# morrislab/rnascan

Hardware: AMD Instinct MI355X
Metric: scored windows/sec (seq+struct, w=12) (higher is better)
Workload: dtype f64

## Files before the change

### include/pfmscan.h

```cpp
#ifndef PFMSCAN_H
#define PFMSCAN_H

#include <stdint.h>

#ifdef __cplusplus
extern "C" {
#endif

#define PFMSCAN_ABI_VERSION 18
#define PFMSCAN_NCODE   8
#define PFMSCAN_SEP     7
#define PFMSCAN_NSTRUCT 7
#define PFMSCAN_MAX_M   64
#define PFMSCAN_MAX_WIDTH 4096
#define PFMSCAN_SITE_GROUP 4096
#define PFMSCAN_SITE_LIMBS 66

#define PFMSCAN_OK          0
#define PFMSCAN_E_BADARG   -1
#define PFMSCAN_E_BADSHAPE -2
#define PFMSCAN_E_OOM      -3
#define PFMSCAN_E_HIP      -4
#define PFMSCAN_E_CAPACITY -5

#define PFMSCAN_PROFILE_NONE 0
#define PFMSCAN_PROFILE_F32  1
#define PFMSCAN_PROFILE_F64  2

typedef struct pfmscan_ctx pfmscan_ctx;
typedef struct pfmscan_motif pfmscan_motif;

int pfmscan_abi_version(void);
// ... 210 lines not shown
                                     int64_t *d_hit_pos, int32_t *d_hit_motif, float *d_hit_seq,
                                     double *d_hit_struct, uint64_t *d_hit_count, void *stream);
int pfmscan_library_hits_letters_host(pfmscan_ctx *ctx, pfmscan_library *lib,
                                      const uint8_t *codes, const uint8_t *codes2, int64_t n_pos,
                                      const double *thr_seq, const double *thr_struct, int64_t capacity,
                                      int64_t *hit_pos, int32_t *hit_motif, float *hit_seq,
                                      double *hit_struct, int64_t *n_hits);
int pfmscan_library_hits_letters_sum_dev(pfmscan_ctx *ctx, pfmscan_library *lib, const uint8_t *d_codes,
                                         const uint8_t *d_codes2, int64_t n_pos, const double *thr_seq,
                                         const double *thr_struct, const double *thr_sum, int64_t capacity,
                                         int64_t *d_hit_pos, int32_t *d_hit_motif, float *d_hit_seq,
                                         double *d_hit_struct, uint64_t *d_hit_count, void *stream);
int pfmscan_library_hits_letters_sum_host(pfmscan_ctx *ctx, pfmscan_library *lib, const uint8_t *codes,
                                          const uint8_t *codes2, int64_t n_pos, const double *thr_seq,
                                          const double *thr_struct, const double *thr_sum, int64_t capacity,
                                          int64_t *hit_pos, int32_t *hit_motif, float *hit_seq,
                                          double *hit_struct, int64_t *n_hits);
int pfmscan_library_letters_sum_thresholds(const double *letter_tables, const double *struct_tables, int n_motifs,
                                           int m, const double *thr_seq, const double *thr_sum, double *thr_eff);

int pfmscan_debug_credit_table(const double *letter_table, int m, double thr_seq, int bits,
                               uint16_t *credits, double *slack);

int pfmscan_debug_library8_credits(const double *letter_table, int m, double thr, uint16_t *credits, double *slack);

int pfmscan_debug_credit8_table(const double *letter_table, int m, double thr, uint16_t *credits, int *mode);

#define PFMSCAN_UPLOAD_RUNTIME 0
#define PFMSCAN_UPLOAD_STAGED  1
int pfmscan_set_upload_mode(pfmscan_ctx *ctx, int mode);
int pfmscan_upload_source_file(pfmscan_ctx *ctx, const void *base, size_t length, const char *path, int64_t file_offset);
int pfmscan_upload_source_file_checked(pfmscan_ctx *ctx, const void *base, size_t length, const char *path,
                                       int64_t file_offset, int64_t st_dev, int64_t st_ino, int64_t st_size);

int pfmscan_dotbracket_annotate_dev(pfmscan_ctx *ctx, const uint8_t *d_in, uint8_t *d_out, int64_t n_pos,
                                    const uint8_t *map, int64_t *d_counts, int64_t *first_bad, void *stream);
int pfmscan_dotbracket_stage(pfmscan_ctx *ctx, const uint8_t *codes, int64_t n_pos, int which, const uint8_t *map,
                             int64_t *counts, int64_t *first_bad);
int pfmscan_dotbracket_annotate_host(pfmscan_ctx *ctx, const uint8_t *in, uint8_t *out, int64_t n_pos,
                                     const uint8_t *map, int64_t *counts, int64_t *first_bad);

#define PFMSCAN_MAX_COVER 1024
#define PFMSCAN_AVG_OK         0
#define PFMSCAN_AVG_DOTBRACKET 1
#define PFMSCAN_AVG_UNCOVERED  2
#define PFMSCAN_AVG_COVER      3
// ... 117 lines not shown
```

### rnascan_amd/_lib.py

```python
import ctypes
import importlib.util
import os
import sys

import numpy as np

HERE = os.path.dirname(os.path.abspath(__file__))
LIB_PATH = os.environ.get("PFMSCAN_LIB") or os.path.join(HERE, "libpfmscan.so")

OK = 0
E_BADARG, E_BADSHAPE, E_OOM, E_HIP, E_CAPACITY = -1, -2, -3, -4, -5
PROFILE_NONE, PROFILE_F32, PROFILE_F64 = 0, 1, 2
SEP = 7
NCODE = 8
NSTRUCT = 7
MAX_M = 64
MAX_WIDTH = 4096
ABI_VERSION = 18

SYMBOLS = [
    "pfmscan_abi_version", "pfmscan_ctx_create", "pfmscan_ctx_destroy", "pfmscan_last_error",
    "pfmscan_device_info", "pfmscan_synchronize", "pfmscan_motif_create", "pfmscan_motif_destroy",
    "pfmscan_pwm_calculate", "pfmscan_scan_dev", "pfmscan_scan_letters_f64_dev", "pfmscan_hits_dev",
    "pfmscan_scan_host", "pfmscan_scan_letters_f64_host", "pfmscan_hits_host", "pfmscan_time_scan_dev",
    "pfmscan_stage", "pfmscan_scan_staged", "pfmscan_hits_staged", "pfmscan_hits_adaptive_dev",
    "pfmscan_library_create", "pfmscan_library_destroy", "pfmscan_library_info", "pfmscan_library_hits_dev",
    "pfmscan_library_hits_staged", "pfmscan_library_hits_host", "pfmscan_library_hits_pipeline_host", "pfmscan_debug_credit_table",
    "pfmscan_library_create_letters", "pfmscan_library_hits_letters_dev", "pfmscan_library_hits_letters_host", "pfmscan_debug_library8_credits",
    "pfmscan_debug_credit8_table",
    "pfmscan_hits_pipeline_host", "pfmscan_staged_positions",
    "pfmscan_hits_letters_f64_dev", "pfmscan_hits_letters_f64_staged", "pfmscan_hits_letters_f64_host",
    "pfmscan_hits_pair_dev", "pfmscan_stage_codes2", "pfmscan_hits_pair_staged", "pfmscan_hits_pair_host", "pfmscan_round_decimals",
    "pfmscan_set_upload_mode", "pfmscan_upload_source_file", "pfmscan_upload_source_file_checked", "pfmscan_fasta_lone_cr", "pfmscan_count_bytes", "pfmscan_fasta_index", "pfmscan_fasta_ids", "pfmscan_gather_spans", "pfmscan_fasta_encode", "pfmscan_tsv_format", "pfmscan_profile_parse", "pfmscan_tsv_number",
    "pfmscan_place_alloc", "pfmscan_place_free", "pfmscan_place_note", "pfmscan_place_trim",
    "pfmscan_dotbracket_annotate_dev", "pfmscan_dotbracket_stage", "pfmscan_dotbracket_annotate_host",
    "pfmscan_average_dev", "pfmscan_average_host", "pfmscan_average_stage", "pfmscan_fragment_ids",
    "pfmscan_profile_colsums_dev", "pfmscan_profile_colsums_host", "pfmscan_profile_colsums_staged",
    "pfmscan_hits_sum_dev", "pfmscan_hits_sum_staged", "pfmscan_hits_sum_host", "pfmscan_hits_sum_pipeline_host",
    "pfmscan_library_hits_sum_dev", "pfmscan_library_hits_sum_staged", "pfmscan_library_hits_sum_host",
    "pfmscan_profile_row_bound_dev", "pfmscan_profile_row_bound_staged", "pfmscan_library_sum_thresholds",
    "pfmscan_site_groups", "pfmscan_site_sums_dev", "pfmscan_site_sums_staged", "pfmscan_site_sums_host",
    "pfmscan_site_groups_lib", "pfmscan_site_order_lib", "pfmscan_site_acc_add", "pfmscan_site_acc_round",
    "pfmscan_site_acc_from_doubles", "pfmscan_site_sums_lib_dev", "pfmscan_site_sums_lib_staged",
    "pfmscan_hits_pair_sum_dev", "pfmscan_hits_pair_sum_staged", "pfmscan_hits_pair_sum_host", "pfmscan_pair_sum_route",
    "pfmscan_debug_round3d", "pfmscan_debug_pair_sum_test", "pfmscan_debug_pair_credits",
    "pfmscan_library_hits_letters_sum_dev", "pfmscan_library_hits_letters_sum_host", "pfmscan_library_letters_sum_thresholds",
    "pfmscan_library_last_launches",
]
PAIR_ROUTE_NONE, PAIR_ROUTE_FUSED, PAIR_ROUTE_TWO_PHASE, PAIR_ROUTE_DENSE, PAIR_ROUTE_CREDITS = range(5)
SITE_GROUP = 4096
SITE_LIMBS = 66
MAX_COVER = 1024
AVG_OK, AVG_DOTBRACKET, AVG_UNCOVERED, AVG_COVER, AVG_BAD_TABLE = range(5)
TSV_CONST, TSV_I64, TSV_F32, TSV_F64, TSV_INDEXED, TSV_FIXED, TSV_WINDOW, TSV_SPAN = range(8)


class TsvColumn(ctypes.Structure):
    _fields_ = [("kind", ctypes.c_int32), ("reserved", ctypes.c_int32), ("data", ctypes.c_void_p),
                ("aux", ctypes.c_void_p), ("blob", ctypes.c_void_p), ("width", ctypes.c_int64)]



class CapacityError(RuntimeError):

    def __init__(self, msg, required):
        RuntimeError.__init__(self, msg)
        self.required = required


_lib = None
# ... 111 lines not shown
    L.pfmscan_place_trim.argtypes = [vp]
    L.pfmscan_place_note.argtypes = [vp]
    L.pfmscan_place_note.restype = ctypes.c_char_p
    L.pfmscan_fasta_index.argtypes = [vp, i64, i64, vp, vp, vp, vp, vp, ctypes.POINTER(i64), i32]
    L.pfmscan_fasta_ids.argtypes = [vp, vp, vp, i64, vp, vp, ctypes.POINTER(i32)]
    L.pfmscan_gather_spans.argtypes = [vp, vp, i64, i32, vp, i64, ctypes.POINTER(i64)]
    L.pfmscan_fasta_encode.argtypes = [vp, vp, vp, vp, i64, i64, vp, i32, vp, vp, i32]
    L.pfmscan_profile_parse.argtypes = [ctypes.c_char_p, i64, i32, i64, vp, ctypes.POINTER(i64)]
    L.pfmscan_tsv_number.argtypes = [vp, i64, i64, vp, i64, ctypes.POINTER(i64), ctypes.POINTER(i64), ctypes.POINTER(i32)]
    L.pfmscan_hits_letters_f64_dev.argtypes = [vp, vp, vp, i64, dbl, i64, vp, vp, vp, vp]
    L.pfmscan_hits_letters_f64_staged.argtypes = [vp, vp, dbl, i64, vp, vp, ctypes.POINTER(i64)]
    L.pfmscan_hits_letters_f64_host.argtypes = [vp, vp, vp, i64, dbl, i64, vp, vp, ctypes.POINTER(i64)]
    L.pfmscan_hits_pair_dev.argtypes = [vp, vp, vp, vp, vp, i64, dbl, dbl, i64, vp, vp, vp, vp, vp]
    L.pfmscan_stage_codes2.argtypes = [vp, vp, i64]
    L.pfmscan_hits_pair_staged.argtypes = [vp, vp, vp, dbl, dbl, i64, vp, vp, vp, ctypes.POINTER(i64)]
    L.pfmscan_hits_pair_host.argtypes = [vp, vp, vp, vp, vp, i64, dbl, dbl, i64, vp, vp, vp, ctypes.POINTER(i64)]
    L.pfmscan_round_decimals.argtypes = [vp, i64, i32, vp, i32]
    L.pfmscan_hits_pair_sum_dev.argtypes = [vp, vp, vp, vp, vp, i64, dbl, dbl, dbl, i64, vp, vp, vp, vp, vp]
    L.pfmscan_hits_pair_sum_staged.argtypes = [vp, vp, vp, dbl, dbl, dbl, i64, vp, vp, vp, ctypes.POINTER(i64)]
    L.pfmscan_hits_pair_sum_host.argtypes = [vp, vp, vp, vp, vp, i64, dbl, dbl, dbl, i64, vp, vp, vp, ctypes.POINTER(i64)]
    L.pfmscan_pair_sum_route.argtypes = [vp]
    L.pfmscan_library_last_launches.argtypes = [vp, ctypes.POINTER(i32), ctypes.POINTER(i32), ctypes.POINTER(i32)]
    L.pfmscan_debug_round3d.argtypes = [vp, i64, vp]
    L.pfmscan_library_hits_letters_sum_dev.argtypes = [vp, vp, vp, vp, i64, vp, vp, vp, i64, vp, vp, vp, vp, vp, vp]
    L.pfmscan_library_hits_letters_sum_host.argtypes = [vp, vp, vp, vp, i64, vp, vp, vp, i64, vp, vp, vp, vp, ctypes.POINTER(i64)]
    L.pfmscan_library_letters_sum_thresholds.argtypes = [vp, vp, i32, i32, vp, vp, vp]
    L.pfmscan_debug_pair_credits.argtypes = [vp, vp, i32, dbl, vp, vp] + [ctypes.POINTER(dbl)] * 4 + [ctypes.POINTER(i32)]
    L.pfmscan_debug_pair_sum_test.argtypes = [vp, vp, i64, dbl, vp, vp, ctypes.POINTER(dbl)]
    L.pfmscan_tsv_format.argtypes = [ctypes.POINTER(TsvColumn), i32, i64, i64, vp, i64, ctypes.POINTER(i64), vp, ctypes.POINTER(i32), i32]
    for name in SYMBOLS:
        if name not in ("pfmscan_ctx_destroy", "pfmscan_motif_destroy", "pfmscan_last_error", "pfmscan_library_destroy",
                        "pfmscan_staged_positions", "pfmscan_place_note"):
            getattr(L, name).restype = i32
    L.pfmscan_staged_positions.restype = i64
    if L.pfmscan_abi_version() != ABI_VERSION:
        raise ImportError("libpfmscan ABI %d, bindings expect %d" % (L.pfmscan_abi_version(), ABI_VERSION))
    _lib = L
    return L


def _ptr(a):
    if a is None:
        return None
    if isinstance(a, np.ndarray):
        return a.ctypes.data_as(ctypes.c_void_p)
    return ctypes.c_void_p(int(a))
# ... 1296 lines not shown
    tj = np.ascontiguousarray(np.broadcast_to(np.asarray(thr_sum, dtype=np.float64), (n,)))
    out = np.empty(n, dtype=np.float64)
    rc = L.pfmscan_library_sum_thresholds(_ptr(T), _ptr(P), n, m, _ptr(ts), _ptr(tj), float(row_sum_max), _ptr(out))
    if rc != OK:
        raise ValueError("pfmscan_library_sum_thresholds: bad argument")
    return out


def library8_credits(letter_table, thr):
    L = load()
    T = np.ascontiguousarray(letter_table, dtype=np.float64)
    if T.ndim != 2 or T.shape[1] != NCODE:
        raise ValueError("letter_table must be [m][8]")
    rows = (T.shape[0] + 3) // 4 * 4
    out = np.zeros((rows, 8), dtype=np.uint16)
    slack = ctypes.c_double(0.0)
    L.pfmscan_debug_library8_credits.argtypes = [ctypes.c_void_p, ctypes.c_int, ctypes.c_double, ctypes.c_void_p, ctypes.POINTER(ctypes.c_double)]
    rc = L.pfmscan_debug_library8_credits(_ptr(T), T.shape[0], float(thr), _ptr(out), ctypes.byref(slack))
    if rc != OK:
        raise ValueError("pfmscan_debug_library8_credits: bad argument")
    return out, slack.value


def credit8_table(letter_table, thr):
    L = load()
    T = np.ascontiguousarray(letter_table, dtype=np.float64)
    if T.ndim != 2 or T.shape[1] != NCODE:
        raise ValueError("letter_table must be [m][8]")
    out = np.zeros((T.shape[0], 8), dtype=np.uint16)
    mode = ctypes.c_int(0)
    rc = L.pfmscan_debug_credit8_table(_ptr(T), T.shape[0], float(thr), _ptr(out), ctypes.byref(mode))
    if rc != OK:
        raise ValueError("pfmscan_debug_credit8_table: bad argument")
    return out, mode.value


def _stream_args(motif, codes, profile):
    if motif.has_letters:
        if codes is None:
            raise ValueError("motif has a letter table: codes required")
        codes = np.ascontiguousarray(codes, dtype=np.uint8)
        n = codes.size
    dt = PROFILE_NONE
    if motif.has_struct:
        if profile is None:
            raise ValueError("motif has a structure PSSM: profile required")
# ... 16 lines not shown
```

### rnascan_amd/csrc/pfmscan_exact.hpp

```cpp
#pragma once
#include <float.h>
#include <math.h>
#include <algorithm>
#include <cmath>
#include <hip/hip_runtime.h>

namespace pfmscan {

constexpr double STRUCT_ROW_MAX = 1024.0;

inline double struct_band(const double *pssm, int m)
{
    double s = 0.0;
    for (int i = 0; i < m * 7; ++i)
        if (std::isfinite(pssm[i])) s += std::fabs(pssm[i]);
    return 24.0 * (double)m * 0x1p-53 * STRUCT_ROW_MAX * s;
}

__device__ __forceinline__ double exact_nan_to_num(double d)
{
    const double c = fmin(fmax(d, -DBL_MAX), DBL_MAX);
    return (d != d) ? 0.0 : c;
}

template <typename ROW_T, typename CellF>
__device__ __forceinline__ double struct_window_rounded(const ROW_T *rows, int m, CellF cell)
{
#pragma clang fp contract(off)
    double score = 0.0;
#pragma unroll 1
    for (int j = 0; j < m; ++j) {
        double d = 0.0;
#pragma unroll 1
        for (int k = 0; k < 7; ++k) {
            const double prod = (double)rows[j * 7 + k] * cell(j, k);
            d = d + prod;
        }
        score = score + exact_nan_to_num(d);
    }
// ... 174 lines not shown
```

### rnascan_amd/csrc/pfmscan_internal.hpp

```cpp
#pragma once
#include <hip/hip_runtime.h>
#include <stdint.h>
#include <atomic>
#include "../../include/pfmscan.h"

namespace pfmscan {

struct CredCache {
    double thr = __builtin_nan("");
    int mode = 0;
    uint16_t cr[16 * 16];
};

struct Cred8Cache {
    double thr = __builtin_nan("");
    int mode = 0;
    uint16_t cr[32 * 8];
};

struct PairCred {
    int mode = 0;
    int m = 0;
    double thr_sum = __builtin_nan("");
    double thr_joint = 0.0, quantum = 0.0, slack = 0.0, survive = 0.0;
// ... 146 lines not shown
    const double *thr_sum;
};
size_t lib_group_bytes(int m, int npair, bool has_struct, int np_bucket);
size_t lib_queue_bytes(int np_bucket);
size_t lib_lds_bytes(int m, int npair, int ng, bool has_struct, int np_bucket);
int lib_np_bucket(int m);
int lib_pick_ng(int np_bucket, int want_groups, int max_groups);
hipError_t launch_library(const LibArgs &a, int n_cu, hipStream_t stream);
constexpr int PROFILE_LETTERS2 = 100;
__host__ __device__ constexpr int lib8_rows(int m) { return (m + 3) / 4 * 4; }
size_t lib8_group_bytes(int m);
size_t lib8_lds_bytes(int m, int ng);
int lib8_pick_ng(int want_groups, int max_groups);
hipError_t launch_library8(const LibArgs &a, int n_cu, hipStream_t stream);

struct ProfLibArgs {
    const void *profile;
    int profile_dtype;
    int64_t n_pos;
    const double *pssm;
    const double *thr;
    double struct_band;
    const int32_t *finite;
    int n_motifs, m, motif_base;
    int64_t pos_offset;
    int64_t capacity;
    int hit_shards;
    int64_t *hit_pos;
    int32_t *hit_motif;
    double *hit_struct;
    unsigned long long *hit_count;
};
hipError_t launch_profile_library(const ProfLibArgs &a, hipStream_t stream);
int64_t profile_library_tile();

hipError_t sort_temp_bytes(int64_t total, int key_bits, size_t *bytes);
hipError_t launch_gather_sorted(const GatherArgs &g, hipStream_t stream);

}
```

### rnascan_amd/csrc/pfmscan_library_api.hip

```cpp
#include <algorithm>
#include <cmath>
#include <cstdlib>
#include <cstring>
#include <new>
#include <string>
#include <vector>

#include "pfmscan_hits.hpp"

using namespace pfmscan;

namespace {

struct LibPass {
    int motif_base = 0, n_real = 0, nmp = 0, ng = 0;
    int ng_real = 0;
    size_t pairs_off = 0;
    size_t letters_off = 0;
    size_t pssm_off = 0;
    size_t thr_off = 0;
};

}

// ... 46 lines not shown
        }
    return q * npair;
}

void pfmscan::pair_sums(const double *T, int m, double *out)
{
    const int npair = (m + 1) / 2;
    for (int t = 0; t < npair; ++t)
        for (int c0 = 0; c0 < 4; ++c0)
            for (int c1 = 0; c1 < 4; ++c1)
                out[t * 16 + (c0 | c1 << 2)] = T[(2 * t) * 8 + c0] + (2 * t + 1 < m ? T[(2 * t + 1) * 8 + c1] : 0.0);
}

struct pfmscan_library {
    pfmscan_ctx *ctx = nullptr;
    int n = 0, m = 0, npair = 0, np_bucket = 8;
    bool has_struct = false;
    bool has_letters = true;
    bool pair = false;
    bool letters8 = false;
    std::vector<double> rows8;
    double *d_pssm_rows = nullptr;
    int32_t *d_finite = nullptr;
    bool all_finite = false;
    double struct_band = 0.0;
    std::vector<double> pairsum;
    std::vector<LibPass> passes;
    uint16_t *d_pairs = nullptr;
    double *d_letters = nullptr, *d_pssm = nullptr, *d_thr = nullptr;
    size_t pairs_elems = 0, thr_elems = 0;
    std::vector<uint16_t> h_pairs;
    std::vector<double> h_thr;
    std::vector<double> cur_seq, cur_struct, eps;
    std::vector<double> h_letters, h_pssm;
    std::vector<double> band;
    std::vector<double> cur_eff, cur_sum;
    bool thr_valid = false;
    int last_launches = 0, last_team_launches = 0, last_max_teams = 0;
};

static int lib_fail(pfmscan_ctx *ctx, int code, const std::string &msg) { return fail(ctx, code, msg); }

extern "C" {

static int create_seq_library(pfmscan_ctx *ctx, const double *letter_tables, const double *struct_pssms, int ncol, int n_motifs, int m,
                              pfmscan_library **out);
// ... 1 lines not shown
int pfmscan_library_create(pfmscan_ctx *ctx, const double *letter_tables, const double *struct_pssms, int n_motifs, int m,
                           pfmscan_library **out)
{
    if (!ctx || !out || (!letter_tables && !struct_pssms)) return lib_fail(ctx, PFMSCAN_E_BADARG, "pfmscan_library_create: NULL argument");
    *out = nullptr;
    if (n_motifs < 1 || n_motifs > 65535) return lib_fail(ctx, PFMSCAN_E_BADSHAPE, "library size outside 1..65535");
    if (m < 1 || m > PFMSCAN_MAX_M)
        return lib_fail(ctx, PFMSCAN_E_BADSHAPE, "PFM width " + std::to_string(m) + " outside 1.." + std::to_string(PFMSCAN_MAX_M));
    if (!letter_tables) {
        HIP_TRY(ctx, hipSetDevice(ctx->device));
        pfmscan_library *lib = new (std::nothrow) pfmscan_library();
        if (!lib) return lib_fail(ctx, PFMSCAN_E_OOM, "out of host memory");
        lib->ctx = ctx;
        lib->n = n_motifs;
        lib->m = m;
        lib->has_struct = true;
        lib->has_letters = false;
        for (int k = 0; k < n_motifs; ++k) lib->struct_band = std::max(lib->struct_band, struct_band(struct_pssms + (size_t)k * m * 7, m));
        std::vector<int32_t> fin((size_t)n_motifs, 1);
        for (int k = 0; k < n_motifs; ++k)
            for (int i = 0; i < m * 7; ++i)
                if (!std::isfinite(struct_pssms[(size_t)k * m * 7 + i])) fin[(size_t)k] = 0;
        if (std::getenv("PFMSCAN_FORCE_GENERIC")) std::fill(fin.begin(), fin.end(), 0);
        const size_t cells = (size_t)n_motifs * m * 7;
        hipError_t e = hipMalloc((void **)&lib->d_pssm_rows, cells * 8);
        if (e == hipSuccess) e = hipMemcpy(lib->d_pssm_rows, struct_pssms, cells * 8, hipMemcpyHostToDevice);
        if (e == hipSuccess) e = hipMalloc((void **)&lib->d_finite, (size_t)n_motifs * 4);
        if (e == hipSuccess) e = hipMemcpy(lib->d_finite, fin.data(), (size_t)n_motifs * 4, hipMemcpyHostToDevice);
        if (e == hipSuccess) e = hipMalloc((void **)&lib->d_thr, (size_t)n_motifs * 8);
        lib->thr_elems = (size_t)n_motifs;
        if (e != hipSuccess) {
            pfmscan_library_destroy(lib);
            return fail_hip(ctx, e, "uploading the library tables");
        }
        *out = lib;
        return PFMSCAN_OK;
    }
    return create_seq_library(ctx, letter_tables, struct_pssms, 7, n_motifs, m, out);
}

}

static int create_seq_library(pfmscan_ctx *ctx, const double *letter_tables, const double *struct_pssms, int ncol, int n_motifs, int m,
                              pfmscan_library **out)
{
    for (int64_t i = 0; i < (int64_t)n_motifs * m; ++i)
        for (int c = 4; c < 8; ++c)
            if (!std::isnan(letter_tables[i * 8 + c]))
// ... 160 lines not shown
{
    if (!ctx || !out || !struct_tables) return lib_fail(ctx, PFMSCAN_E_BADARG, "pfmscan_library_create_letters: NULL argument");
    *out = nullptr;
    if (n_motifs < 1 || n_motifs > 65535) return lib_fail(ctx, PFMSCAN_E_BADSHAPE, "library size outside 1..65535");
    if (m < 1 || m > PFMSCAN_MAX_M)
        return lib_fail(ctx, PFMSCAN_E_BADSHAPE, "PFM width " + std::to_string(m) + " outside 1.." + std::to_string(PFMSCAN_MAX_M));
    for (int64_t i = 0; i < (int64_t)n_motifs * m; ++i)
        if (!std::isnan(struct_tables[i * 8 + 7]))
            return lib_fail(ctx, PFMSCAN_E_BADSHAPE, "column 7 of every letter table must be NaN (the foreign code)");
    if (seq_tables) return create_seq_library(ctx, seq_tables, struct_tables, 8, n_motifs, m, out);
    return create_letters8_library(ctx, struct_tables, n_motifs, m, out);
}

void pfmscan_library_destroy(pfmscan_library *lib)
{
    if (!lib) return;
    if (lib->ctx) (void)hipSetDevice(lib->ctx->device);
    if (lib->d_pairs) (void)hipFree(lib->d_pairs);
    if (lib->d_letters) (void)hipFree(lib->d_letters);
    if (lib->d_pssm) (void)hipFree(lib->d_pssm);
    if (lib->d_thr) (void)hipFree(lib->d_thr);
    if (lib->d_pssm_rows) (void)hipFree(lib->d_pssm_rows);
    if (lib->d_finite) (void)hipFree(lib->d_finite);
    delete lib;
}

int pfmscan_debug_credit_table(const double *letter_table, int m, double thr_seq, int bits, uint16_t *credits, double *slack)
{
    if (!letter_table || !credits || m < 1 || m > PFMSCAN_MAX_M || std::isnan(thr_seq)) return PFMSCAN_E_BADARG;
    if (bits == 0) bits = lib_credit_bits(lib_np_bucket(m));
    if (bits != 10 && bits != 16) return PFMSCAN_E_BADARG;
    const int npair = (m + 1) / 2;
    std::vector<double> ps((size_t)npair * 16);
    pair_sums(letter_table, m, ps.data());
    const double s = build_credits(ps.data(), npair, thr_seq, credits, bits);
    if (slack) *slack = s;
    return PFMSCAN_OK;
}

int pfmscan_debug_library8_credits(const double *letter_table, int m, double thr, uint16_t *credits, double *slack)
{
    if (!letter_table || !credits || m < 1 || m > 32 || std::isnan(thr)) return PFMSCAN_E_BADARG;
    const int rows = lib8_rows(m);
    std::vector<double> r8((size_t)rows * 8, 0.0);
    for (int j = 0; j < m; ++j)
        for (int c = 0; c < 8; ++c) r8[(size_t)j * 8 + c] = std::isnan(letter_table[j * 8 + c]) ? -INFINITY : letter_table[j * 8 + c];
    const double s = build_credits(r8.data(), rows, thr, credits, 16, 8);
    if (slack) *slack = s;
    return PFMSCAN_OK;
}

int pfmscan_library_info(const pfmscan_library *lib, int *n_motifs, int *m, int *n_passes, int *motifs_per_pass, double *max_eps)
{
    if (!lib) return PFMSCAN_E_BADARG;
    if (n_motifs) *n_motifs = lib->n;
    if (m) *m = lib->m;
    const bool tabled = lib->has_letters || lib->letters8;
    if (n_passes) *n_passes = tabled ? (int)lib->passes.size() : 1;
    if (motifs_per_pass) *motifs_per_pass = !tabled ? lib->n : (lib->passes.empty() ? 0 : lib->passes[0].nmp);
    if (max_eps) {
        double mx = 0.0;
        for (double v : lib->eps) mx = std::max(mx, v);
        *max_eps = lib->thr_valid ? mx : NAN;
    }
    return PFMSCAN_OK;
}

int pfmscan_library_last_launches(const pfmscan_library *lib, int *n_launches, int *n_team_launches, int *max_teams)
{
    if (!lib) return PFMSCAN_E_BADARG;
    if (n_launches) *n_launches = lib->last_launches;
// ... 161 lines not shown
                a.capacity = sink.shard_cap;
                a.hit_shards = sink.shards;
                a.hit_pos = sink.pos;
                a.hit_motif = sink.motif;
                a.hit_seq = nullptr;
                a.hit_struct = sink.st;
                a.hit_count = sink.count;
                hipError_t e = launch_library8(a, ctx->n_cu, st);
                if (e != hipSuccess) return fail_hip(ctx, e, "launch k_library8");
                lib_note_launch(lib, 1);
            }
        return PFMSCAN_OK;
    }
    if (!lib->has_letters) {
        ProfLibArgs a;
        std::memset(&a, 0, sizeof(a));
        a.profile = d_profile;
        a.profile_dtype = profile_dtype;
        a.n_pos = n_pos;
        a.pssm = lib->d_pssm_rows;
        a.thr = lib->d_thr;
        a.struct_band = lib->struct_band;
        a.finite = lib->d_finite;
        a.n_motifs = lib->n;
        a.m = lib->m;
        a.motif_base = 0;
        a.pos_offset = pos_offset;
        a.capacity = sink.shard_cap;
        a.hit_shards = sink.shards;
        a.hit_pos = sink.pos;
        a.hit_motif = sink.motif;
        a.hit_struct = sink.st;
        a.hit_count = sink.count;
        hipError_t e = launch_profile_library(a, st);
        if (e != hipSuccess) return fail_hip(ctx, e, "launch k_profile_lib");
        lib_note_launch(lib, 1);
        return PFMSCAN_OK;
    }
    const LibPass &first_pass = lib->passes[0];
    bool teams = lib->has_struct && !lib->pair && lib->passes.size() > 1 && n_pos >= (int64_t)8 * ctx->n_cu * LIB_SEG &&
                 ctx->n_cu >= 16 && !std::getenv("PFMSCAN_LIB_SEQUENTIAL");
    for (const LibPass &ps : lib->passes) teams = teams && ps.ng == first_pass.ng;
    const int64_t max_span = (int64_t)1 << 31;
    for (int64_t base = 0; base < n_pos; base += max_span) {
        const int64_t span_segs = (std::min<int64_t>(max_span, n_pos - base) + LIB_SEG - 1) / LIB_SEG;
        const size_t per_launch = teams && span_segs >= ctx->n_cu ? 4 : 1;
// ... 424 lines not shown
```

### rnascan_amd/csrc/pfmscan_proflib.hip

```cpp
#include <float.h>
#include <math.h>

#include "pfmscan_internal.hpp"
#include "pfmscan_exact.hpp"
#include "pfmscan_hitqueue.hpp"

namespace pfmscan {

constexpr int PL_LANES = 256;
constexpr int PL_GROUPS = 4;
constexpr int PL_BLOCK = PL_LANES * PL_GROUPS;
#ifndef PL_V_OVERRIDE
#define PL_V_OVERRIDE 5
#endif
constexpr int PL_V = PL_V_OVERRIDE;
constexpr int PL_NS = PL_V + 1;
constexpr int PL_UNROLL = (PL_NS % 2) ? 2 * PL_NS : PL_NS;
constexpr int PL_TILE = PL_LANES * PL_V;
#ifndef PL_WAIT_FIRST
#define PL_WAIT_FIRST 1
#endif
#ifndef PL_STAGGER
#define PL_STAGGER 0
#endif
#ifndef PL_INTERLEAVE
#define PL_INTERLEAVE 0
#endif
constexpr int PL_QCAP = 128;

typedef uint32_t pl_u32x4 __attribute__((ext_vector_type(4)));
typedef double pl_f64x2 __attribute__((ext_vector_type(2)));

__device__ __forceinline__ double pl_nan_to_num(double d)
{
    double c = fmin(fmax(d, -DBL_MAX), DBL_MAX);
    return (d != d) ? 0.0 : c;
}

__host__ __device__ constexpr int pl_tile_vals(int m) { return ((PL_TILE + m) * 7 + 3) / 4 * 4; }
__host__ __device__ constexpr int pl_tile_bytes(int m) { return pl_tile_vals(m) * 8; }
__host__ __device__ constexpr int pl_queue_bytes() { return (PL_BLOCK / 64) * PL_QCAP * (8 + 4); }

__device__ __forceinline__ double pl_window_slow(const double *tile, int local, const double *__restrict__ pssm, int m)
{
    double score = 0.0;
#pragma unroll 1
    for (int j = 0; j < m; ++j) {
        const double *r = tile + (local + j) * 7;
        double d = r[0] * pssm[j * 7];
#pragma unroll 1
        for (int k = 1; k < 7; ++k) d = fma(r[k], pssm[j * 7 + k], d);
        score += pl_nan_to_num(d);
    }
    return score;
}

template <bool FINITE>
__device__ __forceinline__ void pl_score_motif(const double *tile, const double *__restrict__ pssm, const double *__restrict__ pssm_next,
                                               int m, int la, double (&acc)[PL_V], double (&P)[7])
{
    constexpr int V = PL_V, NS = PL_NS;
    const volatile __attribute__((address_space(3))) double *vt = (const volatile __attribute__((address_space(3))) double *)tile;
    double rows[NS][7];
#pragma unroll
// ... 47 lines not shown
            }
        }
    };
    int j0 = 0;
#pragma unroll 1
    for (; j0 + PL_UNROLL <= m; j0 += PL_UNROLL) {
#pragma unroll
        for (int uu = 0; uu < PL_UNROLL; ++uu) step(uu, j0 + uu);
    }
#pragma unroll
    for (int uu = 0; uu < PL_UNROLL - 1; ++uu) {
        if (j0 + uu < m) step(uu, j0 + uu);
    }
    if (m & 1) {
#pragma unroll
        for (int k = 0; k < 7; ++k) P[k] = Q[k];
    }
    if (FINITE) {
#pragma unroll
        for (int v = 0; v < V; ++v)
            if (!(fabs(acc[v]) <= DBL_MAX)) acc[v] = pl_window_slow(tile, la + v, pssm, m);
    }
}

template <typename PROF_T>
__global__ __launch_bounds__(PL_BLOCK) void k_profile_lib(const ProfLibArgs a)
{
    constexpr int V = PL_V;
    constexpr int PER = 16 / (int)sizeof(PROF_T);
    typedef PROF_T vec_t __attribute__((ext_vector_type(PER)));
    extern __shared__ __align__(16) unsigned char smem[];
    const int m = a.m;
    double *tile = reinterpret_cast<double *>(smem);
    const int lane = threadIdx.x & 63;
    const int wave = __builtin_amdgcn_readfirstlane(threadIdx.x >> 6);
    const int group = wave / (PL_LANES / 64);
    double *q_sc = reinterpret_cast<double *>(smem + pl_tile_bytes(m)) + wave * PL_QCAP;
    uint32_t *q_wm = reinterpret_cast<uint32_t *>(smem + pl_tile_bytes(m) + (PL_BLOCK / 64) * PL_QCAP * 8) + wave * PL_QCAP;
    const int64_t n_pos = a.n_pos;
    const int64_t tile0 = (int64_t)blockIdx.x * PL_TILE;

    {
        const int nval = pl_tile_vals(m);
        const int64_t e0 = tile0 * 7, e_end = n_pos * 7;
        const PROF_T *__restrict__ src = reinterpret_cast<const PROF_T *>(a.profile) + e0;
        for (int i = threadIdx.x * PER; i < nval; i += PL_BLOCK * PER) {
            double d[PER];
            if (e0 + i + PER <= e_end) {
                const vec_t v = __builtin_nontemporal_load(reinterpret_cast<const vec_t *>(src + i));
#pragma unroll
                for (int e = 0; e < PER; ++e) d[e] = (double)v[e];
            } else {
#pragma unroll
                for (int e = 0; e < PER; ++e) d[e] = (e0 + i + e < e_end) ? (double)src[i + e] : 0.0;
            }
#pragma unroll
            for (int e = 0; e < PER; e += 2) *reinterpret_cast<pl_f64x2 *>(tile + i + e) = pl_f64x2{d[e], d[e + 1]};
        }
    }
    if (threadIdx.x < PL_LANES / 64)
        reinterpret_cast<uint32_t *>(smem + pl_tile_bytes(m) + pl_queue_bytes())[threadIdx.x] = PL_GROUPS;
    __syncthreads();
#if PL_STAGGER
    if (group == 1) __builtin_amdgcn_s_sleep(PL_STAGGER);
    if (group == 2) __builtin_amdgcn_s_sleep(2 * PL_STAGGER);
    if (group == 3) __builtin_amdgcn_s_sleep(3 * PL_STAGGER);
#endif

    const HitShard shard{a.hit_count, a.hit_shards, a.capacity};
    const unsigned long long shard_off = shard.off();
    int qn = 0;
    auto flush = [&]() {
        __builtin_amdgcn_fence(__ATOMIC_RELEASE, "wavefront");
        __builtin_amdgcn_wave_barrier();
        __builtin_amdgcn_fence(__ATOMIC_ACQUIRE, "wavefront");
        const unsigned long long base = shard.reserve_wave(qn);
        for (int i = lane; i < qn; i += 64) {
            const unsigned long long slot = base + (unsigned long long)i;
            if (shard.in_range(slot)) {
                const uint32_t wm = q_wm[i];
                a.hit_pos[shard_off + slot] = tile0 + (int64_t)(wm >> 16) + a.pos_offset;
                a.hit_motif[shard_off + slot] = a.motif_base + (int32_t)(wm & 0xFFFFu);
                a.hit_struct[shard_off + slot] = q_sc[i];
            }
        }
        __builtin_amdgcn_fence(__ATOMIC_RELEASE, "wavefront");
        __builtin_amdgcn_wave_barrier();
        qn = 0;
    };

    const int la = (threadIdx.x & (PL_LANES - 1)) * V;
    const int64_t live_all = n_pos - m + 1 - tile0;
    const int live_n = live_all < 0 ? 0 : (live_all > PL_TILE ? PL_TILE : (int)live_all);
    const __attribute__((address_space(4))) double *thr = (const __attribute__((address_space(4))) double *)a.thr;
    const __attribute__((address_space(4))) int32_t *finite = (const __attribute__((address_space(4))) int32_t *)a.finite;

    uint32_t *ticket = reinterpret_cast<uint32_t *>(smem + pl_tile_bytes(m) + pl_queue_bytes()) + (wave & (PL_LANES / 64 - 1));
    auto draw = [&]() -> uint32_t {
        uint32_t v = 0;
        if (lane == 0) v = atomicAdd(ticket, 1u);
        return v;
    };
    const int nm = a.n_motifs;
    int k = group;
    int kn = nm;
    double P[7];
    int fin = 0;
    if (k < nm) {
        const __attribute__((address_space(4))) double *p0 = (const __attribute__((address_space(4))) double *)(a.pssm + (size_t)k * m * 7);
#pragma unroll
        for (int c = 0; c < 7; ++c) P[c] = p0[c];
        fin = finite[k];
        kn = (int)__builtin_amdgcn_readfirstlane(draw());
    }
#pragma unroll 1
    while (k < nm) {
        const double *pssm = a.pssm + (size_t)k * m * 7;
        const int kc = kn < nm ? kn : k;
        const double *pssm_next = a.pssm + (size_t)kc * m * 7;
        const double t = thr[k];
        const int fin_next = finite[kc];
        double acc[V];
        if (fin)
            pl_score_motif<true>(tile, pssm, pssm_next, m, la, acc, P);
        else
            pl_score_motif<false>(tile, pssm, pssm_next, m, la, acc, P);
        fin = fin_next;
        const double t_lo = t - a.struct_band, t_hi = t + a.struct_band;
        bool maybe[V], any = false;
#pragma unroll
        for (int v = 0; v < V; ++v) {
            maybe[v] = (la + v < live_n) && (acc[v] > t_lo);
            any = any || maybe[v];
        }
        if (__builtin_expect(__builtin_amdgcn_ballot_w64(any) != 0, 0)) {
#pragma unroll
            for (int v = 0; v < V; ++v) {
                bool pass = maybe[v];
                if (__builtin_amdgcn_ballot_w64(pass) == 0) continue;
                if (pass && acc[v] <= t_hi) {
                    acc[v] = struct_window_rounded(tile + (la + v) * 7, m, [&](int j, int c) { return pssm[j * 7 + c]; });
                    pass = acc[v] > t;
                }
                const unsigned long long mk = __builtin_amdgcn_ballot_w64(pass);
                if (mk) {
                    if (qn + 64 > PL_QCAP) flush();
                    if (pass) {
                        const int slot = qn + (int)__builtin_amdgcn_mbcnt_hi((uint32_t)(mk >> 32), __builtin_amdgcn_mbcnt_lo((uint32_t)mk, 0u));
                        q_sc[slot] = acc[v];
                        q_wm[slot] = ((uint32_t)(la + v) << 16) | (uint32_t)k;
                    }
                    qn += __popcll(mk);
                }
            }
        }
        k = kn;
        if (kn < nm) kn = (int)__builtin_amdgcn_readfirstlane(draw());
    }
    if (qn > 0) flush();
}

int64_t profile_library_tile() { return PL_TILE; }

hipError_t launch_profile_library(const ProfLibArgs &a, hipStream_t stream)
{
    if (a.n_pos <= 0 || a.n_motifs <= 0) return hipSuccess;
    if (a.n_motifs > 65536 || a.m < 1 || a.m > PFMSCAN_MAX_M) return hipErrorInvalidValue;
    const unsigned grid = (unsigned)((a.n_pos + PL_TILE - 1) / PL_TILE);
    const size_t lds = (size_t)pl_tile_bytes(a.m) + pl_queue_bytes() + 16;
    static std::atomic<uint64_t> done_f{0}, done_d{0};
    if (a.profile_dtype == PFMSCAN_PROFILE_F64) {
        hipError_t e = allow_dynamic_lds(reinterpret_cast<const void *>(k_profile_lib<double>), done_d, 160 * 1024);
        if (e != hipSuccess) return e;
        hipLaunchKernelGGL(k_profile_lib<double>, dim3(grid), dim3(PL_BLOCK), lds, stream, a);
    } else {
        hipError_t e = allow_dynamic_lds(reinterpret_cast<const void *>(k_profile_lib<float>), done_f, 160 * 1024);
        if (e != hipSuccess) return e;
        hipLaunchKernelGGL(k_profile_lib<float>, dim3(grid), dim3(PL_BLOCK), lds, stream, a);
    }
    return hipGetLastError();
}

}
```

Measured before the change: 151.8 billion.

## Add f32 screening pass with rigorous error bound to skip f64 struct scoring

Adds a float32 screening pass over the profile-library kernel. Each tile also gets an f32 copy of the structure profile in LDS, and each motif gets a host-computed error-bound coefficient, so a motif whose screened scores cannot exceed the threshold is skipped without the f64 scoring loop. An adaptive rule turns the screen off for a wave when most screens end up needing the f64 rerun. The cost is extra LDS use (which may lower occupancy), extra tile-conversion work, and a duplicate pass for motifs that survive the screen.

```diff
diff --git a/include/pfmscan.h b/include/pfmscan.h
--- a/include/pfmscan.h
+++ b/include/pfmscan.h
@@ -7,7 +7,7 @@
 extern "C" {
 #endif
 
-#define PFMSCAN_ABI_VERSION 18
+#define PFMSCAN_ABI_VERSION 19
 #define PFMSCAN_NCODE   8
 #define PFMSCAN_SEP     7
 #define PFMSCAN_NSTRUCT 7
@@ -264,6 +264,9 @@
 int pfmscan_debug_credit_table(const double *letter_table, int m, double thr_seq, int bits,
                                uint16_t *credits, double *slack);
 
+int pfmscan_debug_proflib_screen(const void *rows, int64_t n_rows, int row_is_f64, const double *pssm, int m,
+                                 float *s32_out, double *acc64_out, double *A_out);
+
 int pfmscan_debug_library8_credits(const double *letter_table, int m, double thr, uint16_t *credits, double *slack);
 
 int pfmscan_debug_credit8_table(const double *letter_table, int m, double thr, uint16_t *credits, int *mode);
diff --git a/rnascan_amd/_lib.py b/rnascan_amd/_lib.py
--- a/rnascan_amd/_lib.py
+++ b/rnascan_amd/_lib.py
@@ -16,7 +16,7 @@
 NSTRUCT = 7
 MAX_M = 64
 MAX_WIDTH = 4096
-ABI_VERSION = 18
+ABI_VERSION = 19
 
 SYMBOLS = [
     "pfmscan_abi_version", "pfmscan_ctx_create", "pfmscan_ctx_destroy", "pfmscan_last_error",
@@ -45,7 +45,7 @@
     "pfmscan_hits_pair_sum_dev", "pfmscan_hits_pair_sum_staged", "pfmscan_hits_pair_sum_host", "pfmscan_pair_sum_route",
     "pfmscan_debug_round3d", "pfmscan_debug_pair_sum_test", "pfmscan_debug_pair_credits",
     "pfmscan_library_hits_letters_sum_dev", "pfmscan_library_hits_letters_sum_host", "pfmscan_library_letters_sum_thresholds",
-    "pfmscan_library_last_launches",
+    "pfmscan_library_last_launches", "pfmscan_debug_proflib_screen",
 ]
 PAIR_ROUTE_NONE, PAIR_ROUTE_FUSED, PAIR_ROUTE_TWO_PHASE, PAIR_ROUTE_DENSE, PAIR_ROUTE_CREDITS = range(5)
 SITE_GROUP = 4096
@@ -203,6 +203,7 @@
     L.pfmscan_pair_sum_route.argtypes = [vp]
     L.pfmscan_library_last_launches.argtypes = [vp, ctypes.POINTER(i32), ctypes.POINTER(i32), ctypes.POINTER(i32)]
     L.pfmscan_debug_round3d.argtypes = [vp, i64, vp]
+    L.pfmscan_debug_proflib_screen.argtypes = [vp, i64, i32, vp, i32, vp, vp, ctypes.POINTER(dbl)]
     L.pfmscan_library_hits_letters_sum_dev.argtypes = [vp, vp, vp, vp, i64, vp, vp, vp, i64, vp, vp, vp, vp, vp, vp]
     L.pfmscan_library_hits_letters_sum_host.argtypes = [vp, vp, vp, vp, i64, vp, vp, vp, i64, vp, vp, vp, vp, ctypes.POINTER(i64)]
     L.pfmscan_library_letters_sum_thresholds.argtypes = [vp, vp, i32, i32, vp, vp, vp]
@@ -1545,6 +1546,24 @@
     return out, slack.value
 
 
+def debug_proflib_screen(rows, pssm):
+    L = load()
+    P = np.ascontiguousarray(pssm, dtype=np.float64)
+    if P.ndim != 2 or P.shape[1] != NSTRUCT:
+        raise ValueError("pssm must be [m][7]")
+    R = np.ascontiguousarray(rows)
+    if R.dtype not in (np.float32, np.float64) or R.ndim != 2 or R.shape[1] != NSTRUCT:
+        raise ValueError("rows must be float32 or float64 [n][7]")
+    n_win = max(0, R.shape[0] - P.shape[0] + 1)
+    s32, acc = np.zeros(n_win, dtype=np.float32), np.zeros(n_win, dtype=np.float64)
+    A = ctypes.c_double(0.0)
+    rc = L.pfmscan_debug_proflib_screen(_ptr(R), R.shape[0], int(R.dtype == np.float64), _ptr(P), P.shape[0], _ptr(s32), _ptr(acc),
+                                        ctypes.byref(A))
+    if rc != OK:
+        raise ValueError("pfmscan_debug_proflib_screen: bad argument")
+    return s32, acc, A.value
+
+
 def credit8_table(letter_table, thr):
     L = load()
     T = np.ascontiguousarray(letter_table, dtype=np.float64)
diff --git a/rnascan_amd/csrc/pfmscan_exact.hpp b/rnascan_amd/csrc/pfmscan_exact.hpp
--- a/rnascan_amd/csrc/pfmscan_exact.hpp
+++ b/rnascan_amd/csrc/pfmscan_exact.hpp
@@ -15,6 +15,54 @@
     for (int i = 0; i < m * 7; ++i)
         if (std::isfinite(pssm[i])) s += std::fabs(pssm[i]);
     return 24.0 * (double)m * 0x1p-53 * STRUCT_ROW_MAX * s;
+}
+
+typedef float scr_f32x2 __attribute__((ext_vector_type(2)));
+
+__host__ __device__ constexpr int screen_roundings(int m) { return 8 * m + 1; }
+__host__ __device__ __forceinline__ double screen_floor(int m) { return (double)screen_roundings(m) * 0x1p-149; }
+
+inline double screen_A(const double *pssm, int m)
+{
+    double s = 0.0;
+    for (int i = 0; i < m * 7; ++i) {
+        const double a = std::fabs(pssm[i]);
+        if (!(a <= (double)FLT_MAX) || (a != 0.0 && a < 0x1p-126)) return INFINITY;
+        s = std::nextafter(s + a, INFINITY);
+    }
+    const double n3 = (double)(screen_roundings(m) + 3);
+    const double c32 = std::nextafter(std::nextafter(n3 * 0x1p-24, INFINITY) * (1.0 + 0x1p-20), INFINITY);
+    const double coef = std::nextafter(c32 + (double)(7 * m + 1) * 0x1p-53, INFINITY);
+    const double A = std::nextafter(coef * s, INFINITY);
+    return std::isfinite(A) ? A : INFINITY;
+}
+
+template <typename T>
+__host__ __device__ __forceinline__ float screen_mag_up(T v)
+{
+    const double a = fabs((double)v);
+    if (!(a <= DBL_MAX)) return INFINITY;
+    float f = (float)a;
+    if ((double)f < a) f = __builtin_bit_cast(float, __builtin_bit_cast(uint32_t, f) + 1u);
+    return f;
+}
+
+__host__ __device__ __forceinline__ void screen_row_fma(scr_f32x2 &acc, const scr_f32x2 (&row)[4], const scr_f32x2 (&c)[4])
+{
+#pragma unroll
+    for (int q = 0; q < 4; ++q) acc = __builtin_elementwise_fma(row[q], c[q], acc);
+}
+__host__ __device__ __forceinline__ float screen_finish(scr_f32x2 acc)
+{
+#pragma clang fp contract(off)
+    return acc.x + acc.y;
+}
+__host__ __device__ __forceinline__ double screen_E(float M, double A, int m) { return fma((double)fmaxf(M, FLT_MIN), A, screen_floor(m)); }
+__host__ __device__ __forceinline__ bool screen_survives(float s32, double E, double t_lo)
+{
+#pragma clang fp contract(off)
+    const double d = (double)s32 + E;
+    return !(d <= t_lo && s32 >= -FLT_MAX);
 }
 
 __device__ __forceinline__ double exact_nan_to_num(double d)
diff --git a/rnascan_amd/csrc/pfmscan_internal.hpp b/rnascan_amd/csrc/pfmscan_internal.hpp
--- a/rnascan_amd/csrc/pfmscan_internal.hpp
+++ b/rnascan_amd/csrc/pfmscan_internal.hpp
@@ -192,6 +192,8 @@
     const double *thr;
     double struct_band;
     const int32_t *finite;
+    const float *pssm32;
+    const double *screen_a;
     int n_motifs, m, motif_base;
     int64_t pos_offset;
     int64_t capacity;
diff --git a/rnascan_amd/csrc/pfmscan_library_api.hip b/rnascan_amd/csrc/pfmscan_library_api.hip
--- a/rnascan_amd/csrc/pfmscan_library_api.hip
+++ b/rnascan_amd/csrc/pfmscan_library_api.hip
@@ -92,6 +92,8 @@
     std::vector<double> rows8;
     double *d_pssm_rows = nullptr;
     int32_t *d_finite = nullptr;
+    float *d_pssm32 = nullptr;
+    double *d_screen_a = nullptr;
     bool all_finite = false;
     double struct_band = 0.0;
     std::vector<double> pairsum;
@@ -139,8 +141,23 @@
             for (int i = 0; i < m * 7; ++i)
                 if (!std::isfinite(struct_pssms[(size_t)k * m * 7 + i])) fin[(size_t)k] = 0;
         if (std::getenv("PFMSCAN_FORCE_GENERIC")) std::fill(fin.begin(), fin.end(), 0);
+        std::vector<float> p32((size_t)n_motifs * m * 8, 0.0f);
+        std::vector<double> scr_a((size_t)n_motifs, INFINITY);
+        for (int k = 0; k < n_motifs; ++k) {
+            const double *P = struct_pssms + (size_t)k * m * 7;
+            if (fin[(size_t)k]) scr_a[(size_t)k] = screen_A(P, m);
+            if (scr_a[(size_t)k] < INFINITY) {
+                fin[(size_t)k] |= 2;
+                for (int j = 0; j < m; ++j)
+                    for (int c = 0; c < 7; ++c) p32[((size_t)k * m + j) * 8 + c] = (float)P[j * 7 + c];
+            }
+        }
         const size_t cells = (size_t)n_motifs * m * 7;
         hipError_t e = hipMalloc((void **)&lib->d_pssm_rows, cells * 8);
+        if (e == hipSuccess) e = hipMalloc((void **)&lib->d_pssm32, p32.size() * 4);
+        if (e == hipSuccess) e = hipMemcpy(lib->d_pssm32, p32.data(), p32.size() * 4, hipMemcpyHostToDevice);
+        if (e == hipSuccess) e = hipMalloc((void **)&lib->d_screen_a, (size_t)n_motifs * 8);
+        if (e == hipSuccess) e = hipMemcpy(lib->d_screen_a, scr_a.data(), (size_t)n_motifs * 8, hipMemcpyHostToDevice);
         if (e == hipSuccess) e = hipMemcpy(lib->d_pssm_rows, struct_pssms, cells * 8, hipMemcpyHostToDevice);
         if (e == hipSuccess) e = hipMalloc((void **)&lib->d_finite, (size_t)n_motifs * 4);
         if (e == hipSuccess) e = hipMemcpy(lib->d_finite, fin.data(), (size_t)n_motifs * 4, hipMemcpyHostToDevice);
@@ -347,6 +364,8 @@
     if (lib->d_thr) (void)hipFree(lib->d_thr);
     if (lib->d_pssm_rows) (void)hipFree(lib->d_pssm_rows);
     if (lib->d_finite) (void)hipFree(lib->d_finite);
+    if (lib->d_pssm32) (void)hipFree(lib->d_pssm32);
+    if (lib->d_screen_a) (void)hipFree(lib->d_screen_a);
     delete lib;
 }
 
@@ -372,6 +391,44 @@
         for (int c = 0; c < 8; ++c) r8[(size_t)j * 8 + c] = std::isnan(letter_table[j * 8 + c]) ? -INFINITY : letter_table[j * 8 + c];
     const double s = build_credits(r8.data(), rows, thr, credits, 16, 8);
     if (slack) *slack = s;
+    return PFMSCAN_OK;
+}
+
+int pfmscan_debug_proflib_screen(const void *rows, int64_t n_rows, int row_is_f64, const double *pssm, int m,
+                                 float *s32_out, double *acc64_out, double *A_out)
+{
+    if (!rows || !pssm || !s32_out || !acc64_out || !A_out || m < 1 || m > PFMSCAN_MAX_M || n_rows < 0) return PFMSCAN_E_BADARG;
+    *A_out = screen_A(pssm, m);
+    std::vector<scr_f32x2> c((size_t)m * 4);
+    for (int j = 0; j < m; ++j)
+        for (int q = 0; q < 4; ++q) {
+            const double lo = pssm[j * 7 + 2 * q], hi = 2 * q + 1 < 7 ? pssm[j * 7 + 2 * q + 1] : 0.0;
+            auto cvt = [](double v) { return std::isfinite(v) && std::fabs(v) > (double)FLT_MAX ? (float)std::copysign(INFINITY, v) : (float)v; };
+            c[(size_t)j * 4 + q] = scr_f32x2{cvt(lo), cvt(hi)};
+        }
+    auto entry = [&](int64_t r, int col) -> double {
+        return row_is_f64 ? static_cast<const double *>(rows)[r * 7 + col] : (double)static_cast<const float *>(rows)[r * 7 + col];
+    };
+    auto entry32 = [&](int64_t r, int col) -> float {
+        if (col >= 7) return 0.0f;
+        const double v = entry(r, col);
+        return std::isfinite(v) && std::fabs(v) > (double)FLT_MAX ? (float)std::copysign(INFINITY, v) : (float)v;
+    };
+    for (int64_t i = 0; i + m <= n_rows; ++i) {
+        scr_f32x2 acc = {0.0f, 0.0f};
+        double acc64 = 0.0;
+        for (int j = 0; j < m; ++j) {
+            scr_f32x2 row[4], cj[4];
+            for (int q = 0; q < 4; ++q) {
+                row[q] = scr_f32x2{entry32(i + j, 2 * q), entry32(i + j, 2 * q + 1)};
+                cj[q] = c[(size_t)j * 4 + q];
+            }
+            screen_row_fma(acc, row, cj);
+            for (int col = 0; col < 7; ++col) acc64 = std::fma(entry(i + j, col), pssm[j * 7 + col], acc64);
+        }
+        s32_out[i] = screen_finish(acc);
+        acc64_out[i] = acc64;
+    }
     return PFMSCAN_OK;
 }
 
@@ -579,6 +636,11 @@
         a.thr = lib->d_thr;
         a.struct_band = lib->struct_band;
         a.finite = lib->d_finite;
+        {
+            static const bool screen_on = !(std::getenv("PFMSCAN_PROFLIB_SCREEN") && std::getenv("PFMSCAN_PROFLIB_SCREEN")[0] == '0');
+            a.pssm32 = screen_on ? lib->d_pssm32 : nullptr;
+            a.screen_a = screen_on ? lib->d_screen_a : nullptr;
+        }
         a.n_motifs = lib->n;
         a.m = lib->m;
         a.motif_base = 0;
diff --git a/rnascan_amd/csrc/pfmscan_proflib.hip b/rnascan_amd/csrc/pfmscan_proflib.hip
--- a/rnascan_amd/csrc/pfmscan_proflib.hip
+++ b/rnascan_amd/csrc/pfmscan_proflib.hip
@@ -40,6 +40,11 @@
 __host__ __device__ constexpr int pl_tile_vals(int m) { return ((PL_TILE + m) * 7 + 3) / 4 * 4; }
 __host__ __device__ constexpr int pl_tile_bytes(int m) { return pl_tile_vals(m) * 8; }
 __host__ __device__ constexpr int pl_queue_bytes() { return (PL_BLOCK / 64) * PL_QCAP * (8 + 4); }
+__host__ __device__ constexpr int pl_tickets_bytes() { return 16; }
+__host__ __device__ constexpr int pl_wavemax_bytes() { return (PL_BLOCK / 64) * 4; }
+__host__ __device__ constexpr int pl_plane32_vecs(int m) { return PL_TILE + m; }
+__host__ __device__ constexpr int pl_tile32_bytes(int m) { return 2 * pl_plane32_vecs(m) * 16; }
+typedef float pl_f32x4 __attribute__((ext_vector_type(4)));
 
 __device__ __forceinline__ double pl_window_slow(const double *tile, int local, const double *__restrict__ pssm, int m)
 {
@@ -133,6 +138,70 @@
             if (!(fabs(acc[v]) <= DBL_MAX)) acc[v] = pl_window_slow(tile, la + v, pssm, m);
     }
 }
+
+__device__ __forceinline__ void pl_screen_motif(const pl_f32x4 *tile32, int plane, const float *__restrict__ p32, const float *__restrict__ p32_next,
+                                                int m, int la, float (&s32)[PL_V], double (&S)[4])
+{
+    constexpr int V = PL_V, NS = PL_NS;
+    const volatile __attribute__((address_space(3))) pl_f32x4 *vt = (const volatile __attribute__((address_space(3))) pl_f32x4 *)tile32;
+    scr_f32x2 rows[NS][4], acc[V];
+    auto load_row = [&](const int slot, const int pos) __attribute__((always_inline)) {
+        const pl_f32x4 lo = vt[pos], hi = vt[plane + pos];
+        rows[slot][0] = scr_f32x2{lo.x, lo.y};
+        rows[slot][1] = scr_f32x2{lo.z, lo.w};
+        rows[slot][2] = scr_f32x2{hi.x, hi.y};
+        rows[slot][3] = scr_f32x2{hi.z, hi.w};
+    };
+#pragma unroll
+    for (int s = 0; s < V; ++s) {
+        load_row(s, la + s);
+        acc[s] = scr_f32x2{0.0f, 0.0f};
+    }
+    double R[4];
+    auto step = [&](const int uu, const int j) __attribute__((always_inline)) {
+        const int u = uu % NS;
+        double (&C)[4] = (uu & 1) ? R : S;
+        double (&N)[4] = (uu & 1) ? S : R;
+        __builtin_amdgcn_s_waitcnt(0xC07F);
+        __builtin_amdgcn_sched_barrier(0);
+        const float *nrow = (j + 1 < m) ? p32 + (j + 1) * 8 : p32_next;
+        const __attribute__((address_space(4))) double *prow = (const __attribute__((address_space(4))) double *)nrow;
+#pragma unroll
+        for (int q = 0; q < 4; ++q) N[q] = prow[q];
+        load_row((u + V) % NS, la + j + V);
+        const scr_f32x2 c[4] = {__builtin_bit_cast(scr_f32x2, C[0]), __builtin_bit_cast(scr_f32x2, C[1]),
+                                __builtin_bit_cast(scr_f32x2, C[2]), __builtin_bit_cast(scr_f32x2, C[3])};
+#pragma unroll
+        for (int v = 0; v < V; ++v) screen_row_fma(acc[v], rows[(u + v) % NS], c);
+    };
+    int j0 = 0;
+#pragma unroll 1
+    for (; j0 + PL_UNROLL <= m; j0 += PL_UNROLL) {
+#pragma unroll
+        for (int uu = 0; uu < PL_UNROLL; ++uu) step(uu, j0 + uu);
+    }
+#pragma unroll
+    for (int uu = 0; uu < PL_UNROLL - 1; ++uu) {
+        if (j0 + uu < m) step(uu, j0 + uu);
+    }
+    if (m & 1) {
+#pragma unroll
+        for (int q = 0; q < 4; ++q) S[q] = R[q];
+    }
+#pragma unroll
+    for (int v = 0; v < V; ++v) s32[v] = screen_finish(acc[v]);
+}
+
+#ifdef PL_SCREEN_STATS
+__device__ unsigned long long pl_screen_stats[3];
+extern "C" void pfmscan_diag_proflib_screen_stats(unsigned long long *out)
+{
+    const unsigned long long zero[3] = {0, 0, 0};
+    (void)hipDeviceSynchronize();
+    (void)hipMemcpyFromSymbol(out, HIP_SYMBOL(pl_screen_stats), sizeof(zero));
+    (void)hipMemcpyToSymbol(HIP_SYMBOL(pl_screen_stats), zero, sizeof(zero));
+}
+#endif
 
 template <typename PROF_T>
 __global__ __launch_bounds__(PL_BLOCK) void k_profile_lib(const ProfLibArgs a)
@@ -151,8 +220,14 @@
     const int64_t n_pos = a.n_pos;
     const int64_t tile0 = (int64_t)blockIdx.x * PL_TILE;
 
+    const bool scr_lib = a.screen_a != nullptr;
+    float *wavemax = reinterpret_cast<float *>(smem + pl_tile_bytes(m) + pl_queue_bytes() + pl_tickets_bytes());
+    float *tile32f = reinterpret_cast<float *>(smem + pl_tile_bytes(m) + pl_queue_bytes() + pl_tickets_bytes() + pl_wavemax_bytes());
+    const int plane = pl_plane32_vecs(m);
+
     {
         const int nval = pl_tile_vals(m);
+        float mag = 0.0f;
         const int64_t e0 = tile0 * 7, e_end = n_pos * 7;
         const PROF_T *__restrict__ src = reinterpret_cast<const PROF_T *>(a.profile) + e0;
         for (int i = threadIdx.x * PER; i < nval; i += PL_BLOCK * PER) {
@@ -167,6 +242,20 @@
             }
 #pragma unroll
             for (int e = 0; e < PER; e += 2) *reinterpret_cast<pl_f64x2 *>(tile + i + e) = pl_f64x2{d[e], d[e + 1]};
+            if (scr_lib) {
+#pragma unroll
+                for (int e = 0; e < PER; ++e) {
+                    const int r = (i + e) / 7, c = (i + e) - r * 7;
+                    if (r < plane) tile32f[((c >> 2) * plane + r) * 4 + (c & 3)] = (float)d[e];
+                    mag = fmaxf(mag, screen_mag_up(d[e]));
+                }
+            }
+        }
+        if (scr_lib) {
+            for (int r = threadIdx.x; r < plane; r += PL_BLOCK) tile32f[(plane + r) * 4 + 3] = 0.0f;
+#pragma unroll
+            for (int o = 32; o > 0; o >>= 1) mag = fmaxf(mag, __shfl_xor(mag, o));
+            if (lane == 0) wavemax[wave] = mag;
         }
     }
     if (threadIdx.x < PL_LANES / 64)
@@ -178,6 +267,12 @@
     if (group == 3) __builtin_amdgcn_s_sleep(3 * PL_STAGGER);
 #endif
 
+    float tile_M = 0.0f;
+    if (scr_lib) {
+#pragma unroll
+        for (int w = 0; w < PL_BLOCK / 64; ++w) tile_M = fmaxf(tile_M, wavemax[w]);
+        tile_M = __builtin_bit_cast(float, __builtin_amdgcn_readfirstlane(__builtin_bit_cast(int, tile_M)));
+    }
     const HitShard shard{a.hit_count, a.hit_shards, a.capacity};
     const unsigned long long shard_off = shard.off();
     int qn = 0;
@@ -216,11 +311,15 @@
     int k = group;
     int kn = nm;
     double P[7];
+    double S[4];
+    int held = 0;
+    const __attribute__((address_space(4))) double *scr_a = (const __attribute__((address_space(4))) double *)a.screen_a;
+    int n_scr = 0, n_rerun = 0;
+#ifdef PL_SCREEN_STATS
+    int n_plain = 0;
+#endif
     int fin = 0;
     if (k < nm) {
-        const __attribute__((address_space(4))) double *p0 = (const __attribute__((address_space(4))) double *)(a.pssm + (size_t)k * m * 7);
-#pragma unroll
-        for (int c = 0; c < 7; ++c) P[c] = p0[c];
         fin = finite[k];
         kn = (int)__builtin_amdgcn_readfirstlane(draw());
     }
@@ -231,11 +330,52 @@
         const double *pssm_next = a.pssm + (size_t)kc * m * 7;
         const double t = thr[k];
         const int fin_next = finite[kc];
+        const bool dense = n_scr >= 4 && 5 * n_rerun > 2 * n_scr;
+        if (scr_lib && (fin & 2) && !dense) {
+            const double A = scr_a[k];
+            const float *p32 = a.pssm32 + (size_t)k * m * 8;
+            if (held != 1) {
+                const __attribute__((address_space(4))) double *s0 = (const __attribute__((address_space(4))) double *)p32;
+#pragma unroll
+                for (int q = 0; q < 4; ++q) S[q] = s0[q];
+            }
+            float s32[V];
+            pl_screen_motif(reinterpret_cast<const pl_f32x4 *>(tile32f), plane, p32, a.pssm32 + (size_t)kc * m * 8, m, la, s32, S);
+            float M_here = tile_M;
+            int m_here = m;
+            asm volatile("" : "+s"(M_here), "+s"(m_here));
+            const double E = screen_E(M_here, A, m_here), t_lo = t - a.struct_band;
+            bool live = false;
+#pragma unroll
+            for (int v = 0; v < V; ++v) live = live || screen_survives(s32[v], E, t_lo);
+            ++n_scr;
+            if (__builtin_amdgcn_ballot_w64(live) == 0) {
+                held = 1;
+                fin = fin_next;
+                k = kn;
+                if (kn < nm) kn = (int)__builtin_amdgcn_readfirstlane(draw());
+                continue;
+            }
+            ++n_rerun;
+#ifdef PL_SCREEN_STATS
+            --n_plain;
+#endif
+            held = 0;
+        }
+        if (held != 2) {
+            const __attribute__((address_space(4))) double *p0 = (const __attribute__((address_space(4))) double *)pssm;
+#pragma unroll
+            for (int c = 0; c < 7; ++c) P[c] = p0[c];
+        }
+#ifdef PL_SCREEN_STATS
+        ++n_plain;
+#endif
         double acc[V];
-        if (fin)
+        if (fin & 1)
             pl_score_motif<true>(tile, pssm, pssm_next, m, la, acc, P);
         else
             pl_score_motif<false>(tile, pssm, pssm_next, m, la, acc, P);
+        held = 2;
         fin = fin_next;
         const double t_lo = t - a.struct_band, t_hi = t + a.struct_band;
         bool maybe[V], any = false;
@@ -269,6 +409,13 @@
         if (kn < nm) kn = (int)__builtin_amdgcn_readfirstlane(draw());
     }
     if (qn > 0) flush();
+#ifdef PL_SCREEN_STATS
+    if (lane == 0) {
+        atomicAdd(&pl_screen_stats[0], (unsigned long long)n_scr);
+        atomicAdd(&pl_screen_stats[1], (unsigned long long)n_rerun);
+        atomicAdd(&pl_screen_stats[2], (unsigned long long)n_plain);
+    }
+#endif
 }
 
 int64_t profile_library_tile() { return PL_TILE; }
@@ -278,7 +425,9 @@
     if (a.n_pos <= 0 || a.n_motifs <= 0) return hipSuccess;
     if (a.n_motifs > 65536 || a.m < 1 || a.m > PFMSCAN_MAX_M) return hipErrorInvalidValue;
     const unsigned grid = (unsigned)((a.n_pos + PL_TILE - 1) / PL_TILE);
-    const size_t lds = (size_t)pl_tile_bytes(a.m) + pl_queue_bytes() + 16;
+    if ((a.pssm32 == nullptr) != (a.screen_a == nullptr)) return hipErrorInvalidValue;
+    const size_t lds = (size_t)pl_tile_bytes(a.m) + pl_queue_bytes() + pl_tickets_bytes() +
+                       (a.screen_a ? (size_t)pl_wavemax_bytes() + pl_tile32_bytes(a.m) : 0);
     static std::atomic<uint64_t> done_f{0}, done_d{0};
     if (a.profile_dtype == PFMSCAN_PROFILE_F64) {
         hipError_t e = allow_dynamic_lds(reinterpret_cast<const void *>(k_profile_lib<double>), done_d, 160 * 1024);
```

Result: no change. 152.0 billion, median of 2 (+0.1%).
